# thu-ml/tianshou

Hardware: AMD Instinct MI355X
Metric: PPO learn() update-steps/sec (minibatch 65536, preprocessing incl.) + GAE transitions/sec; cpu_baseline / rocm_eager_baseline are PORTS of the reference path (oracle/), kind=port (higher is better)
Workload: dtype f32; 1 GPU; C2 PPO MuJoCo-shape rollout (BASELINE configs[1]): ONE rollout of 512 envs x 2048 steps = 2^20 transitions, minibatch 65536, obs 17, act 6, MLP[64,64] actor-critic, repeat 10, recompute_advantage off; parallelism=dp1, exchange=none

## Files before the change

### tianshou_amd/csrc/ts_ppo.hip

```cpp
#include <cstdlib>

#include "ts_common.h"

namespace {

using f32x16 = __attribute__((ext_vector_type(16))) float;
using f32x4 = __attribute__((ext_vector_type(4))) float;

constexpr int HID = 64;
constexpr int W2_PITCH = 68;
constexpr int W2_SIZE = HID * W2_PITCH;
constexpr int ACT_PAD = 8;
constexpr int TILE_PITCH = 36;
constexpr int TILE_SIZE = 32 * TILE_PITCH;
constexpr int STEP_THREADS = 256;
constexpr int STEP_WAVES = STEP_THREADS / 64;
constexpr int N_EXTRA = 2;

__device__ __forceinline__ int featF(int r, int h) { return (r & 3) + 8 * (r >> 2) + 4 * h; }

__device__ __forceinline__ f32x16 mfma32(float a, float b, f32x16 c) {
    return __builtin_amdgcn_mfma_f32_32x32x2f32(a, b, c, 0, 0, 0);
}

struct Dims {
    int obs, act;
    int a_w1, a_b1, a_w2, a_b2, a_wmu, a_bmu, a_sig, p_actor;
    int c_w1, c_b1, c_w2, c_b2, c_wv, c_bv, p_total;
};

__host__ __device__ inline Dims make_dims(int obs, int act) {
    Dims d;
    d.obs = obs; d.act = act;
    d.a_w1 = 0;
    d.a_b1 = d.a_w1 + HID * obs;
    d.a_w2 = d.a_b1 + HID;
    d.a_b2 = d.a_w2 + HID * HID;
    d.a_wmu = d.a_b2 + HID;
    d.a_bmu = d.a_wmu + act * HID;
    d.a_sig = d.a_bmu + act;
    d.p_actor = d.a_sig + act;
    d.c_w1 = d.p_actor;
    d.c_b1 = d.c_w1 + HID * obs;
    d.c_w2 = d.c_b1 + HID;
    d.c_b2 = d.c_w2 + HID * HID;
    d.c_wv = d.c_b2 + HID;
    d.c_bv = d.c_wv + HID;
    d.p_total = d.c_bv + 1;
    return d;
}

template <int KS1, int NN>
struct Lds {
    static constexpr int W2 = 0;
    static constexpr int W1 = W2 + NN * W2_SIZE;
    static constexpr int W1_NET = 2 * KS1 * HID;
    static constexpr int B2 = W1 + NN * W1_NET;
    static constexpr int WH = B2 + NN * HID;
    static constexpr int WH_NET = 2 * 2 * 16 * ACT_PAD;
    static constexpr int SMALL = WH + NN * WH_NET;
    static constexpr int END = SMALL + 32;
};

template <int NT, int COUNT, typename SrcFn, typename DstFn>
__device__ __forceinline__ void stage_batch(const float* __restrict__ params, float* lds, SrcFn src, DstFn dst) {
    constexpr int PER = (COUNT + NT - 1) / NT;
    float v[PER];
    int ok[PER];
#pragma unroll
    for (int k = 0; k < PER; ++k) {
        const int idx = threadIdx.x + NT * k;
        const int sidx = src(idx < COUNT ? idx : COUNT - 1);
        ok[k] = (idx < COUNT) & (sidx >= 0);
        v[k] = params[sidx >= 0 ? sidx : 0];
    }
#pragma unroll
    for (int k = 0; k < PER; ++k) v[k] = ok[k] ? v[k] : 0.f;
#pragma unroll
    for (int k = 0; k < PER; ++k) {
        const int idx = threadIdx.x + NT * k;
        if (idx < COUNT) lds[dst(idx)] = v[k];
    }
}

template <int KS1, int NN, int NT>
__device__ __forceinline__ void stage_weights(float* lds, const float* __restrict__ params,
                                              const Dims& d, int first_net) {
    using L = Lds<KS1, NN>;
    constexpr int N_W2 = HID * HID, N_W1 = 2 * KS1 * HID, N_B2 = HID, N_WH = L::WH_NET;
    constexpr int PER_NET = N_W2 + N_W1 + N_B2 + N_WH;
    constexpr int COUNT = NN * PER_NET + 32;
    const int obs = d.obs, act = d.act;
    auto src = [&](int idx) -> int {
        if (idx >= NN * PER_NET) {
            const int i = idx - NN * PER_NET;
            if (i < 8) return i < act ? d.a_bmu + i : -1;
            if (i < 24) return (i & 7) < act ? d.a_sig + (i & 7) : -1;
            return i == 24 ? d.c_bv : -1;
        }
        const int slot = idx / PER_NET;
        int i = idx - slot * PER_NET;
        const int net = first_net + slot;
        if (i < N_W2) return (net ? d.c_w2 : d.a_w2) + i;
        i -= N_W2;
        if (i < N_W1) {
            const int k = i >> 6, row = i & 63;
            const int w1 = net ? d.c_w1 : d.a_w1, b1 = net ? d.c_b1 : d.a_b1;
            return k < obs ? w1 + row * obs + k : (k == obs ? b1 + row : -1);
        }
        i -= N_W1;
        if (i < N_B2) return (net ? d.c_b2 : d.a_b2) + i;
        i -= N_B2;
        const int a = i & 7, r = (i >> 3) & 15, t = (i >> 7) & 1, h = (i >> 8) & 1;
        const int f = 32 * t + featF(r, h);
        if (net == 0) return a < act ? d.a_wmu + a * HID + f : -1;
        return a == 0 ? d.c_wv + f : -1;
    };
    auto dst = [&](int idx) -> int {
        if (idx >= NN * PER_NET) return L::SMALL + (idx - NN * PER_NET);
        const int slot = idx / PER_NET;
        int i = idx - slot * PER_NET;
        if (i < N_W2) return L::W2 + slot * W2_SIZE + (i >> 6) * W2_PITCH + (i & 63);
        i -= N_W2;
        if (i < N_W1) return L::W1 + slot * L::W1_NET + i;
        i -= N_W1;
        if (i < N_B2) return L::B2 + slot * HID + i;
        i -= N_B2;
        return L::WH + slot * L::WH_NET + i;
    };
    stage_batch<NT, COUNT>(params, lds, src, dst);
}

template <int KS1, int NN>
__device__ __forceinline__ void finish_small(float* lds) {
    using L = Lds<KS1, NN>;
    const int i = threadIdx.x;
    if (i >= 8 && i < 24) {
        const float sigma = expf(lds[L::SMALL + i]);
        lds[L::SMALL + i] = (i < 16) ? 1.f / (2.f * (sigma * sigma)) : logf(sigma);
    }
}

template <int KS1, int NT>
__device__ __forceinline__ void stage_image(float* lds, const float* __restrict__ img, int tid = threadIdx.x) {
    constexpr int N4 = Lds<KS1, 1>::END / 4, PER = (N4 + NT - 1) / NT;
    static_assert(Lds<KS1, 1>::END % 4 == 0, "image size");
    f32x4 v[PER];
#pragma unroll
    for (int k = 0; k < PER; ++k) {
        const int q = tid + NT * k;
        v[k] = reinterpret_cast<const f32x4*>(img)[q < N4 ? q : N4 - 1];
    }
#pragma unroll
    for (int k = 0; k < PER; ++k) {
        const int q = tid + NT * k;
        if (q < N4) reinterpret_cast<f32x4*>(lds)[q] = v[k];
    }
}

template <int KS1>
__global__ __launch_bounds__(256) void ppo_build_image_kernel(const float* __restrict__ params, Dims d,
                                                              float* __restrict__ image, int* __restrict__ inv) {
    using L = Lds<KS1, 1>;
    const int net = blockIdx.x;
    float* img = image + net * L::END;
    for (int i = threadIdx.x; i < L::END; i += 256) img[i] = 0.f;
    __syncthreads();
    stage_weights<KS1, 1, 256>(img, params, d, net);
    __syncthreads();
    finish_small<KS1, 1>(img);
    if (!inv) return;
    constexpr int N_W2 = HID * HID, N_W1 = 2 * KS1 * HID, N_B2 = HID, N_WH = L::WH_NET;
    constexpr int PER_NET = N_W2 + N_W1 + N_B2 + N_WH;
    for (int idx = threadIdx.x; idx < PER_NET + 32; idx += 256) {
        int src = -1, dst = -1;
        if (idx >= PER_NET) {
            const int i = idx - PER_NET;
            if (net == 0 && i < 8 && i < d.act) { src = d.a_bmu + i; dst = L::SMALL + i; }
            if (net == 1 && i == 24) { src = d.c_bv; dst = L::SMALL + 24; }
        } else {
            int i = idx;
            if (i < N_W2) { src = (net ? d.c_w2 : d.a_w2) + i; dst = L::W2 + (i >> 6) * W2_PITCH + (i & 63); }
            else if ((i -= N_W2) < N_W1) {
                const int k = i >> 6, row = i & 63;
                if (k < d.obs) src = (net ? d.c_w1 : d.a_w1) + row * d.obs + k;
                else if (k == d.obs) src = (net ? d.c_b1 : d.a_b1) + row;
                dst = L::W1 + i;
            } else if ((i -= N_W1) < N_B2) { src = (net ? d.c_b2 : d.a_b2) + i; dst = L::B2 + i; }
            else {
                i -= N_B2;
                const int a = i & 7, r = (i >> 3) & 15, t = (i >> 7) & 1, h = (i >> 8) & 1;
                const int f = 32 * t + featF(r, h);
                if (net == 0) { if (a < d.act) src = d.a_wmu + a * HID + f; }
                else if (a == 0) src = d.c_wv + f;
                dst = L::WH + i;
            }
        }
        if (src >= 0) inv[src] = net * L::END + dst;
    }
}

__device__ __forceinline__ float fast_tanh(float x) {
    const float e = __builtin_amdgcn_exp2f(x * 2.885390081777927f);
    return 1.f - 2.f * __builtin_amdgcn_rcpf(e + 1.f);
}

#ifndef TS_PK
#define TS_PK 2
#endif
using f32x2 = __attribute__((ext_vector_type(2))) float;
__device__ __forceinline__ void tanh16(f32x16& a) {
#if TS_PK < 1
#pragma unroll
    for (int r = 0; r < 16; ++r) a[r] = fast_tanh(a[r]);
    return;
#endif
#pragma unroll
    for (int r = 0; r < 16; r += 2) {
        const f32x2 x = {a[r], a[r + 1]};
        const f32x2 y = x * 2.885390081777927f;
        f32x2 e = {__builtin_amdgcn_exp2f(y[0]), __builtin_amdgcn_exp2f(y[1])};
        e = e + 1.f;
        const f32x2 q = {__builtin_amdgcn_rcpf(e[0]), __builtin_amdgcn_rcpf(e[1])};
        const f32x2 t = 1.f - 2.f * q;
        a[r] = t[0];
        a[r + 1] = t[1];
    }
}

__device__ __forceinline__ void dtanh16(f32x16& v, const f32x16& hh) {
#if TS_PK < 2
#pragma unroll
    for (int r = 0; r < 16; ++r) v[r] = v[r] * (1.f - hh[r] * hh[r]);
    return;
#endif
#pragma unroll
    for (int r = 0; r < 16; r += 2) {
        const f32x2 hv = {hh[r], hh[r + 1]};
        const f32x2 g = {v[r], v[r + 1]};
        const f32x2 o = g * (1.f - hv * hv);
        v[r] = o[0];
        v[r + 1] = o[1];
    }
}

template <int KS1, int NN>
__device__ __forceinline__ void trunk_forward(const float* lds, int net, const float (&x)[KS1],
                                              int i, int h, f32x16 (&h1)[2], f32x16 (&h2)[2]) {
    using L = Lds<KS1, NN>;
    const float* w1 = lds + L::W1 + net * L::W1_NET;
    const float* w2 = lds + L::W2 + net * W2_SIZE;
    const float* b2 = lds + L::B2 + net * HID;
#pragma unroll
    for (int t = 0; t < 2; ++t) {
        f32x16 acc = {0.f, 0.f, 0.f, 0.f, 0.f, 0.f, 0.f, 0.f, 0.f, 0.f, 0.f, 0.f, 0.f, 0.f, 0.f, 0.f};
#pragma unroll
        for (int s = 0; s < KS1; ++s) acc = mfma32(w1[(KS1 * h + s) * HID + 32 * t + i], x[s], acc);
        tanh16(acc);
        h1[t] = acc;
    }
#pragma unroll
    for (int t2 = 0; t2 < 2; ++t2) {
        f32x16 acc;
#pragma unroll
        for (int g = 0; g < 4; ++g) {
            const f32x4 b = *reinterpret_cast<const f32x4*>(b2 + 32 * t2 + 8 * g + 4 * h);
            acc[4 * g + 0] = b[0]; acc[4 * g + 1] = b[1]; acc[4 * g + 2] = b[2]; acc[4 * g + 3] = b[3];
        }
#pragma unroll
        for (int t = 0; t < 2; ++t) {
#pragma unroll
            for (int g = 0; g < 4; ++g) {
                const f32x4 a = *reinterpret_cast<const f32x4*>(w2 + (32 * t2 + i) * W2_PITCH + 32 * t + 8 * g + 4 * h);
#pragma unroll
                for (int q = 0; q < 4; ++q) acc = mfma32(a[q], h1[t][4 * g + q], acc);
            }
            __builtin_amdgcn_sched_barrier(0);
        }
        tanh16(acc);
        h2[t2] = acc;
    }
}

template <int KS1, int NN, int NA>
__device__ __forceinline__ void head_forward(const float* lds, int net, int h, const f32x16 (&h2)[2],
                                             float (&out)[NA]) {
    using L = Lds<KS1, NN>;
    const float* wh = lds + L::WH + net * L::WH_NET + h * (2 * 16 * ACT_PAD);
#pragma unroll
    for (int a = 0; a < NA; ++a) out[a] = 0.f;
#pragma unroll
    for (int t = 0; t < 2; ++t) {
#pragma unroll
        for (int r = 0; r < 16; ++r) {
            const float* p = wh + (t * 16 + r) * ACT_PAD;
            if constexpr (NA == 1) {
                out[0] += h2[t][r] * p[0];
            } else {
                const f32x4 w0 = *reinterpret_cast<const f32x4*>(p);
                const f32x4 w1 = *reinterpret_cast<const f32x4*>(p + 4);
#pragma unroll
                for (int a = 0; a < 4; ++a) {
                    out[a] += h2[t][r] * w0[a];
                    if (a + 4 < NA) out[a + 4] += h2[t][r] * w1[a];
                }
            }
            if (NA > 1 && (r & 7) == 7) __builtin_amdgcn_sched_barrier(0);
        }
    }
#pragma unroll
    for (int a = 0; a < NA; ++a) out[a] += __shfl_xor(out[a], 32, 64);
}

template <int KS1>
__device__ __forceinline__ void load_x(const float* __restrict__ obs, int64_t row, int obs_dim, int h,
                                       float (&x)[KS1]) {
#pragma unroll
    for (int s = 0; s < KS1; ++s) {
        const int k = KS1 * h + s;
        float v = 0.f;
        if (k < obs_dim) v = obs[row * obs_dim + k];
        else if (k == obs_dim) v = 1.f;
        x[s] = v;
    }
}

constexpr float LOG_SQRT_2PI = 0.91893853320467274178f;

__device__ __forceinline__ float gaussian_logp(const float (&mu)[ACT_PAD], const float (&act)[ACT_PAD],
                                               const float* sm, int act_dim) {
    float lp = 0.f;
#pragma unroll
    for (int a = 0; a < ACT_PAD; ++a) {
        if (a < act_dim) {
            const float dlt = act[a] - mu[a];
            lp += -(dlt * dlt) * sm[8 + a] - sm[16 + a] - LOG_SQRT_2PI;
        }
    }
    return lp;
}

template <int KS1>
__global__ __launch_bounds__(512) void ppo_infer_kernel(const float* __restrict__ params, Dims d,
                                                        const float* __restrict__ obs,
                                                        const float* __restrict__ act, int64_t n,
                                                        float* __restrict__ v_out,
                                                        float* __restrict__ logp_out,
                                                        float* __restrict__ mu_out, float mu_bound) {
    extern __shared__ __attribute__((aligned(16))) float lds[];
    using L = Lds<KS1, 2>;
    stage_weights<KS1, 2, 512>(lds, params, d, 0);
    __syncthreads();
    finish_small<KS1, 2>(lds);
    __syncthreads();
    const int lane = threadIdx.x & 63, i = lane & 31, h = lane >> 5;
    const int wave = threadIdx.x >> 6, waves = blockDim.x >> 6;
    const int64_t n_tiles = (n + 31) / 32;
    for (int64_t tile = (int64_t)blockIdx.x * waves + wave; tile < n_tiles; tile += (int64_t)gridDim.x * waves) {
        const int64_t srow = tile * 32 + i;
        const bool valid = srow < n;
        const int64_t row = valid ? srow : n - 1;
        float x[KS1];
        load_x<KS1>(obs, row, d.obs, h, x);
        f32x16 h1[2], h2[2];
        if (v_out) {
            trunk_forward<KS1, 2>(lds, 1, x, i, h, h1, h2);
            float v[1];
            head_forward<KS1, 2, 1>(lds, 1, h, h2, v);
            if (valid && h == 0) v_out[srow] = v[0] + lds[L::SMALL + 24];
        }
        if (logp_out || mu_out) {
            trunk_forward<KS1, 2>(lds, 0, x, i, h, h1, h2);
            float mu[ACT_PAD], a[ACT_PAD];
            head_forward<KS1, 2, ACT_PAD>(lds, 0, h, h2, mu);
#pragma unroll
            for (int k = 0; k < ACT_PAD; ++k) {
                mu[k] += lds[L::SMALL + k];
                if (mu_bound > 0.f) mu[k] = mu_bound * fast_tanh(mu[k]);
                a[k] = (logp_out && k < d.act) ? act[row * d.act + k] : 0.f;
            }
            if (mu_out && valid && h == 0) {
#pragma unroll
                for (int k = 0; k < ACT_PAD; ++k)
                    if (k < d.act) mu_out[srow * d.act + k] = mu[k];
            }
            if (logp_out) {
                const float lp = gaussian_logp(mu, a, lds + L::SMALL, d.act);
                if (valid && h == 0) logp_out[srow] = lp;
            }
        }
    }
}

struct StepArgs {
    const float* params;
    const float* rec;
    int rec_w;
    const int64_t* rows;
    int64_t n_rows;
    float inv_batch;
    const float* adv_stats;
    float eps_clip, dual_clip, vf_coef, ent_coef;
    int value_clip, adv_norm, a2c;
    int nets;
    float mu_bound;
    const float* image;
    float* slabs;
    int slab_w;
    long long* dbg;
};

#ifdef TS_PHASE_MARKS
#define TS_MARK(g, k)                                                                  \
    do {                                                                               \
        if ((g).dbg && blockIdx.x == 0 && threadIdx.x == 0) (g).dbg[(k)] = (long long)__builtin_readcyclecounter(); \
        if ((g).dbg && threadIdx.x == 0 && ((k) == 0 || (k) == 17))                    \
            (g).dbg[64 + 2 * blockIdx.x + ((k) == 17)] = (long long)__builtin_amdgcn_s_memrealtime();    \
        if ((g).dbg && threadIdx.x == 0 && (k) == 0)       \
            (g).dbg[64 + 1024 + blockIdx.x] = ((long long)__builtin_amdgcn_s_getreg((4 - 1) << 11 | 0 << 6 | 20) << 32) | \
                                              (unsigned)__builtin_amdgcn_s_getreg((32 - 1) << 11 | 0 << 6 | 4);          \
    } while (0)
#else
#define TS_MARK(g, k) do { } while (0)
#endif

__device__ __forceinline__ void tile_write(float* tile, const f32x16& v, int j, int h) {
#pragma unroll
    for (int r = 0; r < 16; ++r) tile[featF(r, h) * TILE_PITCH + j] = v[r];
}

__device__ __forceinline__ void wave_lds_sync() {
    __builtin_amdgcn_fence(__ATOMIC_ACQ_REL, "wavefront");
    __builtin_amdgcn_wave_barrier();
}

template <int KS1>
struct TileIn {
    float x[KS1];
    float act[ACT_PAD];
    float adv, logp_old, ret, v_old;
    float w;
};

template <int KS1>
struct RecFetch {
    static constexpr int N = (32 * ((2 * KS1 + 14) / 4) + 63) / 64;
    f32x4 v[N];
    float w;
};

struct RowId { int64_t id; float w; };

__device__ __forceinline__ RowId row_fetch(const StepArgs& g, int64_t tile, int lane) {
    const int i = lane & 31;
    const int64_t srow = tile * 32 + i;
    const bool valid = srow < g.n_rows;
    const int64_t pos = valid ? srow : g.n_rows - 1;
    RowId r;
    r.id = g.rows ? g.rows[pos] : pos;
    r.w = valid ? g.inv_batch : 0.f;
    return r;
}

template <int KS1>
__device__ __forceinline__ RecFetch<KS1> rec_fetch(const StepArgs& g, const RowId& row, int lane) {
    RecFetch<KS1> f;
    constexpr int REC_FETCH = RecFetch<KS1>::N;
    f.w = row.w;
    const int parts = g.rec_w >> 2;
    const int total = 32 * parts;
    const int lo = (int)(row.id & 0xffffffffLL), hi = (int)(row.id >> 32);
#pragma unroll
    for (int k = 0; k < REC_FETCH; ++k) {
        int q = lane + 64 * k;
        q = q < total ? q : total - 1;
        const int rec = q / parts, part = q - rec * parts;
        const int64_t rid = ((int64_t)__shfl(hi, rec, 64) << 32) | (uint32_t)__shfl(lo, rec, 64);
        f.v[k] = *reinterpret_cast<const f32x4*>(g.rec + rid * g.rec_w + part * 4);
    }
    return f;
}

template <int KS1>
__device__ __forceinline__ TileIn<KS1> rec_commit(const RecFetch<KS1>& f, const StepArgs& g, const Dims& d,
                                                   float* rb, int lane) {
    constexpr int REC_FETCH = RecFetch<KS1>::N;
    const int i = lane & 31, h = lane >> 5;
    const int parts = g.rec_w >> 2;
    const int total = 32 * parts;
#pragma unroll
    for (int k = 0; k < REC_FETCH; ++k) {
        const int q = lane + 64 * k;
        if (q < total) *reinterpret_cast<f32x4*>(rb + q * 4) = f.v[k];
    }
    wave_lds_sync();
    TileIn<KS1> t;
    const float* r = rb + i * g.rec_w;
#pragma unroll
    for (int s = 0; s < KS1; ++s) {
        const int k = KS1 * h + s;
        float v = 0.f;
        if (k < d.obs) v = r[k];
        else if (k == d.obs) v = 1.f;
        t.x[s] = v;
    }
#pragma unroll
    for (int k = 0; k < ACT_PAD; ++k) t.act[k] = (k < d.act) ? r[d.obs + k] : 0.f;
    const float* aux = r + d.obs + d.act;
    t.adv = aux[0];
    t.ret = aux[1];
    t.logp_old = aux[2];
    t.v_old = aux[3];
    t.w = f.w;
    wave_lds_sync();
    return t;
}

constexpr int P128 = 132;
constexpr int T2_FLOATS = 128 * P128;
constexpr int T2_XROW = 64;
constexpr int MISC_ROWS = 9;
constexpr int MISC_SLOT = MISC_ROWS * 64;
constexpr int T2_MISC = 96 * P128;
static_assert(T2_MISC + STEP_WAVES * MISC_SLOT <= T2_FLOATS, "misc slots must fit behind the phase-B tiles");

struct Slab2 {
    int w1[2], w2[2], b2[2], head[2], hb[2], sig, loss, width;
};

__host__ __device__ inline Slab2 slab2_layout(int act, int kp) {
    Slab2 L;
    int o = 0;
    for (int n = 0; n < 2; ++n) {
        const int n_head = n ? 1 : act;
        L.w1[n] = o; o += HID * kp;
        L.w2[n] = o; o += HID * HID;
        L.b2[n] = o; o += HID;
        L.head[n] = o; o += n_head * HID;
        L.hb[n] = o; o += n_head;
        if (n == 0) { L.sig = o; o += act; }
    }
    L.loss = o; o += N_EXTRA;
    L.width = (o + 3) & ~3;
    return L;
}

__device__ __forceinline__ int slab_col_to_param(int col, const Dims& d, int kp) {
    const Slab2 L = slab2_layout(d.act, kp);
    if (col >= L.loss) return col < L.loss + N_EXTRA ? d.p_total + (col - L.loss) : -1;
    const int n = col >= L.w1[1];
    const int c = col - L.w1[n];
    if (c < HID * kp) {
        const int f = c / kp, k = c - f * kp;
        const int w1 = n ? d.c_w1 : d.a_w1, b1 = n ? d.c_b1 : d.a_b1;
        return k < d.obs ? w1 + f * d.obs + k : (k == d.obs ? b1 + f : -1);
    }
    return (n ? d.c_w2 : d.a_w2) + (c - HID * kp);
}

__device__ __forceinline__ f32x4 ld4(const float* p) { return *reinterpret_cast<const f32x4*>(p); }

__device__ __forceinline__ void tile128_write(float* T, int row0, const f32x16& v, int col, int h) {
#pragma unroll
    for (int r = 0; r < 16; ++r) T[(row0 + featF(r, h)) * P128 + col] = v[r];
}

using gfloat_ptr = __attribute__((address_space(1))) float*;
#ifndef TS_SLAB_PLAIN_STORES
__device__ __forceinline__ void slab_st(float* p, float v) {
    __hip_atomic_store((gfloat_ptr)p, v, __ATOMIC_RELAXED, __HIP_MEMORY_SCOPE_AGENT);
}
#else
__device__ __forceinline__ void slab_st(float* p, float v) { *(gfloat_ptr)p = v; }
#endif

__device__ __forceinline__ void store_acc(float* p, float v, bool first) {
    if (!first) v += *(gfloat_ptr)p;
    slab_st(p, v);
}

template <bool WANT_RSUM>
__device__ __forceinline__ f32x16 tile128_mma(const float* T, int rowA, int rowB, int i, int h, float* rsum) {
    f32x16 c = {0.f, 0.f, 0.f, 0.f, 0.f, 0.f, 0.f, 0.f, 0.f, 0.f, 0.f, 0.f, 0.f, 0.f, 0.f, 0.f};
    const float* pa = T + (rowA + i) * P128 + 16 * h;
    const float* pb = T + (rowB + i) * P128 + 16 * h;
    float rs = 0.f;
    f32x4 a[4], b[4];
#pragma unroll
    for (int q = 0; q < 4; ++q) { a[q] = ld4(pa + 4 * q); b[q] = ld4(pb + 4 * q); }
#pragma unroll
    for (int ch = 0; ch < 4; ++ch) {
        f32x4 an[4], bn[4];
        if (ch < 3) {
#pragma unroll
            for (int q = 0; q < 4; ++q) { an[q] = ld4(pa + 32 * (ch + 1) + 4 * q); bn[q] = ld4(pb + 32 * (ch + 1) + 4 * q); }
        }
#pragma unroll
        for (int q = 0; q < 4; ++q) {
#pragma unroll
            for (int e = 0; e < 4; ++e) c = mfma32(a[q][e], b[q][e], c);
            if (WANT_RSUM) rs += (a[q][0] + a[q][1]) + (a[q][2] + a[q][3]);
        }
        if (ch < 3) {
#pragma unroll
            for (int q = 0; q < 4; ++q) { a[q] = an[q]; b[q] = bn[q]; }
        }
    }
    if (WANT_RSUM) *rsum = rs + __shfl_xor(rs, 32, 64);
    return c;
}

template <int KS1, bool ACTOR, bool BOUNDED = false>
__device__ __forceinline__ void net_fwd_bwd(float* lds, float* scratch, const StepArgs& g, const Dims& d,
                                            const TileIn<KS1>& in, int lane_in, f32x16 (&h1)[2], f32x16 (&h2)[2],
                                            f32x16 (&dz1)[2], float (&gw)[ACTOR ? ACT_PAD : 1], float& misc) {
    using L = Lds<KS1, 1>;
    int lane = lane_in;
    asm volatile("" : "+v"(lane));
    [[maybe_unused]] constexpr int MK = ACTOR ? 2 : 10;
    constexpr int NA = ACTOR ? ACT_PAD : 1;
    const int i = lane & 31, h = lane >> 5;
    trunk_forward<KS1, 1>(lds, 0, in.x, i, h, h1, h2);
    TS_MARK(g, MK + 0);

    float dout[NA];
    const float w = in.w;
    const float* sm = lds + L::SMALL;
    float* Qt = scratch;
    if constexpr (ACTOR) {
        float mu[ACT_PAD];
        head_forward<KS1, 1, ACT_PAD>(lds, 0, h, h2, mu);
        const f32x4 b0 = ld4(sm), b1 = ld4(sm + 4), v0 = ld4(sm + 8), v1 = ld4(sm + 12), s0 = ld4(sm + 16), s1 = ld4(sm + 20);
        float dlt[ACT_PAD], inv_var[ACT_PAD];
        [[maybe_unused]] float bgrad[ACT_PAD];
        constexpr bool bounded = BOUNDED;
        float logp = 0.f;
        int n_act = d.act;
        asm volatile("" : "+s"(n_act));
#pragma unroll
        for (int k = 0; k < ACT_PAD; ++k) {
            const float bm = k < 4 ? b0[k & 3] : b1[k & 3], iv = k < 4 ? v0[k & 3] : v1[k & 3], ls = k < 4 ? s0[k & 3] : s1[k & 3];
            float m = mu[k] + bm;
            if (bounded) {
                const float t = fast_tanh(m);
                m = g.mu_bound * t;
                bgrad[k] = 1.f - t * t;
            }
            dlt[k] = in.act[k] - m;
            inv_var[k] = 2.f * iv;
            logp += -(dlt[k] * dlt[k]) * iv - ls - (k < n_act ? LOG_SQRT_2PI : 0.f);
        }
        float mean = 0.f, den = 1.f;
        if (g.adv_norm) { mean = g.adv_stats[0]; den = g.adv_stats[1] + 1e-8f; }
        const float A = (in.adv - mean) / den;
        const bool a2c = g.a2c != 0;
        const float ratio = a2c ? 1.f : expf(logp - in.logp_old);
        const float surr1 = ratio * A;
        const float lo = 1.f - g.eps_clip, hi = 1.f + g.eps_clip;
        const float surr2 = fminf(fmaxf(ratio, lo), hi) * A;
        const float clip1 = fminf(surr1, surr2);
        float basek = (surr1 <= surr2) ? A : 0.f;
        const float dA = g.dual_clip * A;
        const bool dual = (g.dual_clip > 0.f) && (A < 0.f);
        float term = dual ? -fmaxf(clip1, dA) : -clip1;
        basek = (dual && !(clip1 >= dA)) ? 0.f : basek;
        term = a2c ? -logp * A : term;
        basek = a2c ? A : basek;
        const float dlogp = -basek * ratio * w;
        const float ent_w = g.ent_coef * w;
        float dsig[ACT_PAD];
#pragma unroll
        for (int k = 0; k < ACT_PAD; ++k) {
            dout[k] = dlogp * dlt[k] * inv_var[k];
            if (bounded) dout[k] = (dout[k] * g.mu_bound) * bgrad[k];
            const float ds = dlogp * (dlt[k] * dlt[k] * inv_var[k] - 1.f) - ent_w;
            dsig[k] = k < n_act ? ds : 0.f;
        }
#pragma unroll
        for (int k = 0; k < ACT_PAD; ++k) Qt[(8 * h + k) * TILE_PITCH + i] = h ? dsig[k] : dout[k];
        if (h == 0) Qt[16 * TILE_PITCH + i] = term * w;
    } else {
        float v[1];
        head_forward<KS1, 1, 1>(lds, 0, h, h2, v);
        const float value = v[0] + sm[24];
        const float ret = in.ret;
        const float vf1 = (ret - value) * (ret - value);
        const float vo = in.v_old;
        const float dvo = value - vo;
        const float vclip = vo + fminf(fmaxf(dvo, -g.eps_clip), g.eps_clip);
        const float vf2 = (ret - vclip) * (ret - vclip);
        const float g1 = -2.f * (ret - value);
        const float g2 = (dvo >= -g.eps_clip && dvo <= g.eps_clip) ? -2.f * (ret - vclip) : 0.f;
        const float dv_clip = (vf1 > vf2) ? g1 : ((vf2 > vf1) ? g2 : 0.5f * (g1 + g2));
        const bool vc = g.value_clip != 0;
        const float term = vc ? fmaxf(vf1, vf2) : vf1;
        const float dv = vc ? dv_clip : g1;
        dout[0] = dv * g.vf_coef * w;
        Qt[(16 * h) * TILE_PITCH + i] = h ? term * w : dout[0];
    }
    wave_lds_sync();
    {
        const int row = lane < 16 ? lane : 16;
        const float* rp = Qt + row * TILE_PITCH;
        f32x4 q[8];
#pragma unroll
        for (int k = 0; k < 8; ++k) q[k] = ld4(rp + 4 * k);
        float sacc = 0.f;
#pragma unroll
        for (int k = 0; k < 8; ++k) sacc += (q[k][0] + q[k][1]) + (q[k][2] + q[k][3]);
        const bool mine = ACTOR ? (lane <= 16) : (lane == 0 || lane == 16);
        misc = mine ? sacc : 0.f;
    }
    wave_lds_sync();
    __builtin_amdgcn_sched_barrier(0);
    TS_MARK(g, MK + 1);
    __builtin_amdgcn_s_setprio(ACTOR ? 2 : 0);

    float* SA = scratch;
    float* SB = scratch + TILE_SIZE;
    tile_write(SA, h2[0], i, h);
    tile_write(SB, h2[1], i, h);
    if (lane < 32) {
        if constexpr (ACTOR) {
            const f32x4 d0 = {dout[0], dout[1], dout[2], dout[3]};
            const f32x4 d1 = {dout[4], dout[5], dout[6], dout[7]};
            *reinterpret_cast<f32x4*>(SA + lane * TILE_PITCH + 32) = d0;
            *reinterpret_cast<f32x4*>(SB + lane * TILE_PITCH + 32) = d1;
        } else {
            SA[lane * TILE_PITCH + 32] = dout[0];
        }
    }
    wave_lds_sync();
    {
        const float* rowp = (lane < 32 ? SA : SB) + (lane & 31) * TILE_PITCH;
#pragma unroll
        for (int a = 0; a < NA; ++a) gw[a] = 0.f;
#pragma unroll 2
        for (int q = 0; q < 8; ++q) {
            const f32x4 hv = ld4(rowp + 4 * q);
#pragma unroll
            for (int e = 0; e < 4; ++e) {
                const int smp = 4 * q + e;
                if constexpr (ACTOR) {
                    const f32x4 d0 = ld4(SA + smp * TILE_PITCH + 32);
                    const f32x4 d1 = ld4(SB + smp * TILE_PITCH + 32);
#pragma unroll
                    for (int a = 0; a < 4; ++a) {
                        gw[a] += d0[a] * hv[e];
                        gw[a + 4] += d1[a] * hv[e];
                    }
                } else {
                    gw[0] += SA[smp * TILE_PITCH + 32] * hv[e];
                }
            }
        }
    }
    wave_lds_sync();
    __builtin_amdgcn_sched_barrier(0);
    TS_MARK(g, MK + 2);

    {
        const float* wh = lds + L::WH + h * (2 * 16 * ACT_PAD);
        [[maybe_unused]] f32x2 d01, d23, d45, d67;
        if constexpr (ACTOR) {
            d01 = f32x2{dout[0], dout[1]}; d23 = f32x2{dout[2], dout[3]};
            d45 = f32x2{dout[4], dout[5]}; d67 = f32x2{dout[6], dout[7]};
        }
#pragma unroll
        for (int t = 0; t < 2; ++t) {
            f32x16 dhv;
#pragma unroll
            for (int r = 0; r < 16; ++r) {
                const float* p = wh + (t * 16 + r) * ACT_PAD;
                if constexpr (ACTOR) {
                    const f32x4 w0 = ld4(p);
                    const f32x4 w1 = ld4(p + 4);
#if TS_PK < 3
                    dhv[r] = dout[0] * w0[0] + dout[1] * w0[1] + dout[2] * w0[2] + dout[3] * w0[3] +
                             dout[4] * w1[0] + dout[5] * w1[1] + dout[6] * w1[2] + dout[7] * w1[3];
                    continue;
#endif
                    f32x2 sacc = d01 * f32x2{w0[0], w0[1]};
                    sacc = d23 * f32x2{w0[2], w0[3]} + sacc;
                    sacc = d45 * f32x2{w1[0], w1[1]} + sacc;
                    sacc = d67 * f32x2{w1[2], w1[3]} + sacc;
                    dhv[r] = sacc[0] + sacc[1];
                } else {
                    dhv[r] = dout[0] * p[0];
                }
                if (ACTOR && (r & 7) == 7) __builtin_amdgcn_sched_barrier(0);
            }
            dtanh16(dhv, h2[t]);
            h2[t] = dhv;
        }
    }

    {
        const float* w2 = lds + L::W2;
#pragma unroll
        for (int t1 = 0; t1 < 2; ++t1) {
            f32x16 accd = {0.f, 0.f, 0.f, 0.f, 0.f, 0.f, 0.f, 0.f, 0.f, 0.f, 0.f, 0.f, 0.f, 0.f, 0.f, 0.f};
#pragma unroll
            for (int t = 0; t < 2; ++t) {
#pragma unroll
                for (int r = 0; r < 16; ++r)
                    accd = mfma32(w2[(32 * t + featF(r, h)) * W2_PITCH + 32 * t1 + i], h2[t][r], accd);
                __builtin_amdgcn_sched_barrier(0);
            }
            dtanh16(accd, h1[t1]);
            dz1[t1] = accd;
        }
    }
    __builtin_amdgcn_sched_barrier(0);
    TS_MARK(g, MK + 3);
}

template <int KS1, bool ACTOR>
__device__ __forceinline__ void net_wgrad(float* lds, const StepArgs& g, const Dims& d, const TileIn<KS1>& in,
                                          const f32x16 (&h1)[2], const f32x16 (&dz2)[2], const f32x16 (&dz1)[2],
                                          const float (&gw)[ACTOR ? ACT_PAD : 1], float misc, int wave, int lane_in,
                                          float* slab, const Slab2& SL, bool first) {
    [[maybe_unused]] constexpr int MK = ACTOR ? 2 : 10;
    constexpr int NA = ACTOR ? ACT_PAD : 1;
    constexpr int net = ACTOR ? 0 : 1;
    constexpr int KP = 2 * KS1;
    int lane = lane_in;
    asm volatile("" : "+v"(lane), "+v"(wave), "+s"(slab));
    const int i = lane & 31, h = lane >> 5;
    const int col = 32 * wave + i;
    float* T = lds;
    __syncthreads();
    tile128_write(T, 0, dz2[0], col, h);
    tile128_write(T, 32, dz2[1], col, h);
    tile128_write(T, 64, h1[0], col, h);
    tile128_write(T, 96, h1[1], col, h);
    __syncthreads();
    TS_MARK(g, MK + 4);
    {
        const int tM = wave >> 1, tN = wave & 1;
        float rs;
        const f32x16 c = tile128_mma<true>(T, 32 * tM, 64 + 32 * tN, i, h, &rs);
        float* p = slab + SL.w2[net] + (32 * tM + 4 * h) * HID + 32 * tN + i;
        if (first) {
#pragma unroll
            for (int r = 0; r < 16; ++r) slab_st(p + ((r & 3) + 8 * (r >> 2)) * HID, c[r]);
        } else {
#pragma unroll
            for (int r = 0; r < 16; ++r) slab_st(p + ((r & 3) + 8 * (r >> 2)) * HID, ((gfloat_ptr)p)[((r & 3) + 8 * (r >> 2)) * HID] + c[r]);
        }
        if (tN == 0 && h == 0) store_acc(slab + SL.b2[net] + 32 * tM + i, rs, first);
    }
    __syncthreads();
    TS_MARK(g, MK + 5);
    tile128_write(T, 0, dz1[0], col, h);
    tile128_write(T, 32, dz1[1], col, h);
#pragma unroll
    for (int s = 0; s < KS1; ++s) T[(T2_XROW + KS1 * h + s) * P128 + col] = in.x[s];
    {
        float* M = T + T2_MISC + wave * MISC_SLOT;
#pragma unroll
        for (int a = 0; a < NA; ++a) M[a * 64 + lane] = gw[a];
        M[8 * 64 + lane] = misc;
    }
    __syncthreads();
    const bool w1_wave = ACTOR ? (wave < 2) : (wave >= 2);
    if (w1_wave) {
        const int tM = wave & 1;
        const f32x16 c = tile128_mma<false>(T, 32 * tM, T2_XROW, i, h, nullptr);
        if (i < KP) {
            float* p = slab + SL.w1[net] + (32 * tM + 4 * h) * KP + i;
            if (first) {
#pragma unroll
                for (int r = 0; r < 16; ++r) slab_st(p + ((r & 3) + 8 * (r >> 2)) * KP, c[r]);
            } else {
#pragma unroll
                for (int r = 0; r < 16; ++r) slab_st(p + ((r & 3) + 8 * (r >> 2)) * KP, ((gfloat_ptr)p)[((r & 3) + 8 * (r >> 2)) * KP] + c[r]);
            }
        }
    } else {
        const int part = wave & 1;
        const float* M = T + T2_MISC;
        const int n_head = ACTOR ? d.act : 1;
        if (ACTOR) {
#pragma unroll
            for (int q = 0; q < 4; ++q) {
                const int row = 4 * part + q;
                float v = 0.f;
#pragma unroll
                for (int sl = 0; sl < STEP_WAVES; ++sl) v += M[sl * MISC_SLOT + row * 64 + lane];
                if (row < n_head) store_acc(slab + SL.head[net] + row * HID + lane, v, first);
            }
        } else if (part == 1) {
            float v = 0.f;
#pragma unroll
            for (int sl = 0; sl < STEP_WAVES; ++sl) v += M[sl * MISC_SLOT + lane];
            store_acc(slab + SL.head[net] + lane, v, first);
        }
        if (part == 0) {
            float v = 0.f;
#pragma unroll
            for (int sl = 0; sl < STEP_WAVES; ++sl) v += M[sl * MISC_SLOT + 8 * 64 + lane];
            if (lane < 8) { if (lane < n_head) store_acc(slab + SL.hb[net] + lane, v, first); }
            else if (lane < 16) { if (ACTOR && lane - 8 < d.act) store_acc(slab + SL.sig + lane - 8, v, first); }
            else if (lane == 16) store_acc(slab + SL.loss + net, v, first);
        }
    }
    TS_MARK(g, MK + 6);
}

template <int KS1, bool BOUNDED = false>
__global__ __launch_bounds__(STEP_THREADS, 2) void ppo_step2_kernel(StepArgs g, Dims d) {
    extern __shared__ __attribute__((aligned(16))) float lds[];
    using L = Lds<KS1, 1>;
    static_assert(L::END + STEP_WAVES * 2 * TILE_SIZE <= T2_FLOATS, "weight image + wave scratch must fit under the tiles");
    const int lane0 = threadIdx.x & 63, wave0 = threadIdx.x >> 6;
    const Slab2 SL = slab2_layout(d.act, 2 * KS1);

    const int64_t n_tiles = (g.n_rows + 31) / 32;
    const int64_t per_iter = (int64_t)gridDim.x * STEP_WAVES;
    const int64_t n_iter = (n_tiles + per_iter - 1) / per_iter;
    const int64_t tile0 = (int64_t)blockIdx.x * STEP_WAVES + wave0;
    float* slab = g.slabs + (int64_t)blockIdx.x * g.slab_w;

    TS_MARK(g, 0);
    for (int64_t it = 0; it < n_iter; ++it) {
        __builtin_amdgcn_s_setprio(3);
        int lane = lane0, wave = wave0;
        asm volatile("" : "+v"(lane), "+v"(wave));
        float* scratch = lds + L::END + wave * (2 * TILE_SIZE);
        const RowId row0 = row_fetch(g, it * per_iter + tile0, lane);
        const RecFetch<KS1> f = rec_fetch<KS1>(g, row0, lane);
        if (it > 0) __syncthreads();
        stage_image<KS1, STEP_THREADS>(lds, g.image, 64 * wave + lane);
        const TileIn<KS1> in = rec_commit<KS1>(f, g, d, scratch, lane);
        __syncthreads();
        TS_MARK(g, 1);
        const bool first = it == 0;
        f32x16 h1[2], h2[2], dz1[2];
        float misc;
        {
            float gw[ACT_PAD];
            net_fwd_bwd<KS1, true, BOUNDED>(lds, scratch, g, d, in, lane, h1, h2, dz1, gw, misc);
            net_wgrad<KS1, true>(lds, g, d, in, h1, h2, dz1, gw, misc, wave, lane, slab, SL, first);
        }
        __syncthreads();
        TS_MARK(g, 18);
        {
            int tid = 64 * wave + lane;
            asm volatile("" : "+v"(tid));
            stage_image<KS1, STEP_THREADS>(lds, g.image + L::END, tid);
        }
        __syncthreads();
        TS_MARK(g, 9);
        __builtin_amdgcn_s_setprio(1);
        {
            float gw[1];
            net_fwd_bwd<KS1, false>(lds, scratch, g, d, in, lane, h1, h2, dz1, gw, misc);
            net_wgrad<KS1, false>(lds, g, d, in, h1, h2, dz1, gw, misc, wave, lane, slab, SL, first);
        }
    }
    TS_MARK(g, 17);
}

template <int KS1, bool BOUNDED = false>
__global__ __launch_bounds__(STEP_THREADS, 2) void ppo_step1_kernel(StepArgs g, Dims d, int net) {
    extern __shared__ __attribute__((aligned(16))) float lds[];
    using L = Lds<KS1, 1>;
    const int lane0 = threadIdx.x & 63, wave0 = threadIdx.x >> 6;
    const Slab2 SL = slab2_layout(d.act, 2 * KS1);

    const int64_t n_tiles = (g.n_rows + 31) / 32;
    const int64_t per_iter = (int64_t)gridDim.x * STEP_WAVES;
    const int64_t n_iter = (n_tiles + per_iter - 1) / per_iter;
    const int64_t tile0 = (int64_t)blockIdx.x * STEP_WAVES + wave0;
    float* slab = g.slabs + (int64_t)blockIdx.x * g.slab_w;
    TS_MARK(g, 0);
    {
        const int z0 = net == 0 ? SL.w1[1] : 0, z1 = net == 0 ? SL.loss : SL.w1[1];
        for (int c = z0 + (int)threadIdx.x; c < z1; c += STEP_THREADS) slab_st(slab + c, 0.f);
        if (threadIdx.x == 0) slab_st(slab + SL.loss + (1 - net), 0.f);
    }
    for (int64_t it = 0; it < n_iter; ++it) {
        __builtin_amdgcn_s_setprio(3);
        int lane = lane0, wave = wave0;
        asm volatile("" : "+v"(lane), "+v"(wave));
        float* scratch = lds + L::END + wave * (2 * TILE_SIZE);
        const RowId row0 = row_fetch(g, it * per_iter + tile0, lane);
        const RecFetch<KS1> f = rec_fetch<KS1>(g, row0, lane);
        if (it > 0) __syncthreads();
        stage_image<KS1, STEP_THREADS>(lds, g.image + (net ? L::END : 0), 64 * wave + lane);
        const TileIn<KS1> in = rec_commit<KS1>(f, g, d, scratch, lane);
        __syncthreads();
        TS_MARK(g, 1);
        const bool first = it == 0;
        f32x16 h1[2], h2[2], dz1[2];
        float misc;
        if (net == 0) {
            float gw[ACT_PAD];
            net_fwd_bwd<KS1, true, BOUNDED>(lds, scratch, g, d, in, lane, h1, h2, dz1, gw, misc);
            net_wgrad<KS1, true>(lds, g, d, in, h1, h2, dz1, gw, misc, wave, lane, slab, SL, first);
        } else {
            float gw[1];
            net_fwd_bwd<KS1, false>(lds, scratch, g, d, in, lane, h1, h2, dz1, gw, misc);
            net_wgrad<KS1, false>(lds, g, d, in, h1, h2, dz1, gw, misc, wave, lane, slab, SL, first);
        }
    }
    TS_MARK(g, 17);
}

#include "ts_ppo_q.h"
#include "ts_npg_q.h"

constexpr int RED_THREADS = 1024;

__global__ __launch_bounds__(RED_THREADS) void ppo_reduce_slabs_kernel(const float* __restrict__ slabs,
                                                                       int n_slabs, int slab_w, Dims d, int kp, int k1q,
                                                                       float* __restrict__ grad,
                                                                       float* __restrict__ sumsq_part,
                                                                       const float* __restrict__ params,
                                                                       float* __restrict__ losses,
                                                                       float* __restrict__ parts) {
    __shared__ float red[RED_THREADS / 64][64];
    const int lane = threadIdx.x & 63, wave = threadIdx.x >> 6;
    const int col = blockIdx.x * 64 + lane;
    const int n_params = d.p_total;
    float s = 0.f;
    if (col < slab_w) {
#pragma unroll 16
        for (int k = wave; k < n_slabs; k += RED_THREADS / 64) s += slabs[(int64_t)k * slab_w + col];
    }
    red[wave][lane] = s;
    __syncthreads();
    if (wave == 0) {
        float t = 0.f;
#pragma unroll
        for (int k = 0; k < RED_THREADS / 64; ++k) t += red[k][lane];
        const int pidx = col < slab_w ? (k1q > 0 ? q4::slab3_col_to_param(col, d, k1q) : slab_col_to_param(col, d, kp)) : -1;
        if (pidx >= 0 && pidx < (parts ? n_params : n_params + N_EXTRA)) grad[pidx] = t;
        if (parts && pidx == n_params) parts[1] = t;
        if (parts && pidx == n_params + 1) parts[2] = t;
        float q = (pidx >= 0 && pidx < n_params) ? t * t : 0.f;
#pragma unroll
        for (int off = 32; off > 0; off >>= 1) q += __shfl_down(q, off, 64);
        if (lane == 0) sumsq_part[blockIdx.x] = q;
        if (parts && blockIdx.x == 0 && lane == 0) parts[0] = 0.f;
        if ((losses || parts) && blockIdx.x == 0 && lane == 0) {
            float ent = 0.f;
            for (int k = 0; k < d.act; ++k)
                ent += 0.5f + 0.5f * 1.8378770664093453f + logf(expf(params[d.a_sig + k]));
            if (losses) losses[3] = ent;
            if (parts) parts[3] = ent;
        }
    }
}

struct AdamArgs {
    float* params;
    float* m;
    float* v;
    const float* grad;
    const float* sumsq_part;
    int n_part, n_params;
    float max_grad_norm, lr_step, bc2_sqrt, beta1, beta2, eps;
    float omb1, omb2;
    float vf_coef, ent_coef;
    int opt_kind, centered;
    float wd, lr, alpha, oma, momentum;
    float* losses;
    int apply;
    float* image;
    const int* inv;
    int sig_off, act, small0;
};

constexpr int ADAM_THREADS = 256;

__global__ __launch_bounds__(ADAM_THREADS) void ppo_adam_kernel(AdamArgs a) {
    __shared__ float red[ADAM_THREADS / 64];
    const int tid = threadIdx.x, lane = tid & 63, wave = tid >> 6;
    const int p = blockIdx.x * ADAM_THREADS + tid;
    const bool mine = a.apply && p < a.n_params;
    const int pc = mine ? p : 0;
    float g_raw = a.grad[pc], m = a.m[pc], v = a.v[pc], par = a.params[pc];
    const int slot = (mine && a.image) ? a.inv[pc] : -1;
    float sq = 0.f;
    if (a.sumsq_part) {
        for (int k = tid; k < a.n_part; k += ADAM_THREADS) sq += a.sumsq_part[k];
    } else {
        for (int q = tid; q < a.n_params; q += ADAM_THREADS) { const float gq = a.grad[q]; sq += gq * gq; }
    }
#pragma unroll
    for (int off = 32; off > 0; off >>= 1) sq += __shfl_down(sq, off, 64);
    if (lane == 0) red[wave] = sq;
    __syncthreads();
    float total = 0.f;
#pragma unroll
    for (int k = 0; k < ADAM_THREADS / 64; ++k) total += red[k];
    const float norm = sqrtf(total);
    float scale = 1.f;
    if (a.max_grad_norm > 0.f) scale = fminf(a.max_grad_norm / (norm + 1e-6f), 1.f);

    if (a.losses && blockIdx.x == 0 && tid == 0) {
        const float clip = a.grad[a.n_params], vf = a.grad[a.n_params + 1];
        const float ent = a.losses[3];
        a.losses[0] = clip + a.vf_coef * vf - a.ent_coef * ent;
        a.losses[1] = clip;
        a.losses[2] = vf;
    }
    if (mine) {
        float gq = g_raw * scale;
        if (a.wd != 0.f) gq = gq + a.wd * par;
        float np_;
        if (a.opt_kind == TS_OPT_RMSPROP) {
            v = v * a.alpha + a.oma * gq * gq;
            float avg;
            if (a.centered) {
                m = m + (gq - m) * a.oma;
                avg = sqrtf(v + -1.f * m * m);
            } else {
                avg = sqrtf(v);
            }
            avg = avg + a.eps;
            if (a.momentum > 0.f) {
                m = m * a.momentum + gq / avg;
                np_ = par + -a.lr * m;
            } else {
                np_ = par + (-a.lr * gq) / avg;
            }
        } else {
            m = m + (gq - m) * a.omb1;
            v = v * a.beta2 + a.omb2 * gq * gq;
            const float denom = sqrtf(v) / a.bc2_sqrt + a.eps;
            np_ = par + (-a.lr_step * m) / denom;
        }
        a.params[p] = np_;
        a.m[p] = m;
        a.v[p] = v;
        if (a.image) {
            if (slot >= 0) a.image[slot] = np_;
            const int k = p - a.sig_off;
            if (k >= 0 && k < a.act) {
                const float sigma = expf(np_);
                a.image[a.small0 + 8 + k] = 1.f / (2.f * (sigma * sigma));
                a.image[a.small0 + 16 + k] = logf(sigma);
            }
        }
    }
}

__global__ __launch_bounds__(256) void ppo_pack_kernel(const float* __restrict__ obs,
                                                       const float* __restrict__ act,
                                                       const float* __restrict__ adv,
                                                       const float* __restrict__ ret,
                                                       const float* __restrict__ logp_old,
                                                       const float* __restrict__ v_old, int64_t n,
                                                       int obs_dim, int act_dim, int rec_w,
                                                       float* __restrict__ rec) {
    const int64_t total = n * rec_w;
    const int64_t stride = (int64_t)gridDim.x * blockDim.x;
    for (int64_t t = (int64_t)blockIdx.x * blockDim.x + threadIdx.x; t < total; t += stride) {
        const int64_t row = t / rec_w;
        const int c = (int)(t - row * rec_w);
        float v = 0.f;
        if (c < obs_dim) v = obs[row * obs_dim + c];
        else if (c < obs_dim + act_dim) v = act[row * act_dim + (c - obs_dim)];
        else if (c == obs_dim + act_dim) v = adv[row];
        else if (c == obs_dim + act_dim + 1) v = ret[row];
        else if (c == obs_dim + act_dim + 2) v = logp_old[row];
        else if (c == obs_dim + act_dim + 3) v = v_old[row];
        rec[t] = v;
    }
}

__global__ __launch_bounds__(1024) void ppo_adv_stats_kernel(const float* __restrict__ adv,
                                                             const int64_t* __restrict__ perm,
                                                             const int64_t* __restrict__ mb_offset,
                                                             float* __restrict__ out) {
    __shared__ double r1[16], r2[16];
    const int64_t lo = mb_offset[blockIdx.x], hi = mb_offset[blockIdx.x + 1];
    double s1 = 0.0, s2 = 0.0;
    for (int64_t k = lo + threadIdx.x; k < hi; k += 1024) {
        const double v = (double)adv[perm ? perm[k] : k];
        s1 += v;
        s2 += v * v;
    }
#pragma unroll
    for (int off = 32; off > 0; off >>= 1) {
        s1 += __shfl_down(s1, off, 64);
        s2 += __shfl_down(s2, off, 64);
    }
    if ((threadIdx.x & 63) == 0) { r1[threadIdx.x >> 6] = s1; r2[threadIdx.x >> 6] = s2; }
    __syncthreads();
    if (threadIdx.x == 0) {
        double t1 = 0.0, t2 = 0.0;
        for (int w = 0; w < 16; ++w) { t1 += r1[w]; t2 += r2[w]; }
        const double n = (double)(hi - lo);
        const double mean = t1 / n;
        const double var = (t2 - n * mean * mean) / (n - 1.0);
        out[2 * blockIdx.x] = (float)mean;
        out[2 * blockIdx.x + 1] = (float)sqrt(var > 0.0 ? var : 0.0);
    }
// ... 774 lines not shown
```

Measured before the change: 15580 update-steps/s.

## Split W1 gradient across all four waves using 16x16x4 MFMA tiles

The first-layer weight gradient used to be computed by two waves with 32x32x2 MFMA while the other two waves did the head and bias reductions. Now every wave computes a 16-row slice of dW1 with 16x16x4 MFMA, which only covers the padded K width instead of a full 32-wide tile. The head and bias reductions are redistributed by wave index. To match the new MFMA operand pattern, the LDS columns for dz1 and X are permuted. The aim is to balance work across waves and cut wasted MFMA lanes, at the cost of more complex LDS indexing and every wave doing both jobs.

```diff
diff --git a/tianshou_amd/csrc/ts_ppo.hip b/tianshou_amd/csrc/ts_ppo.hip
--- a/tianshou_amd/csrc/ts_ppo.hip
+++ b/tianshou_amd/csrc/ts_ppo.hip
@@ -21,6 +21,10 @@
 
 __device__ __forceinline__ f32x16 mfma32(float a, float b, f32x16 c) {
     return __builtin_amdgcn_mfma_f32_32x32x2f32(a, b, c, 0, 0, 0);
+}
+
+__device__ __forceinline__ f32x4 mfma16x4(float a, float b, f32x4 c) {
+    return __builtin_amdgcn_mfma_f32_16x16x4f32(a, b, c, 0, 0, 0);
 }
 
 struct Dims {
@@ -610,6 +614,43 @@
     return c;
 }
 
+__device__ __forceinline__ int dw1_col(int col) { return (col & ~15) | ((col & 1) << 3) | ((col & 15) >> 1); }
+
+template <int KS1>
+__device__ __forceinline__ void dw1_wave(const float* T, int wave, int lane, float* w1, bool first) {
+    constexpr int KP = 2 * KS1;
+    constexpr int NT = KP > 16 ? 2 : 1;
+    static_assert(KP <= 32 && T2_XROW + 16 * NT <= 96, "X^T rows stay below the misc slots");
+    const int m = lane & 15, kg = lane >> 4;
+    const int s0 = 16 * (kg & 1) + 8 * (kg >> 1);
+    const float* pa = T + (16 * wave + m) * P128 + s0;
+    const float* pb = T + (T2_XROW + m) * P128 + s0;
+    f32x4 acc[NT];
+#pragma unroll
+    for (int n = 0; n < NT; ++n) acc[n] = f32x4{0.f, 0.f, 0.f, 0.f};
+#pragma unroll
+    for (int t = 0; t < 8; ++t) {
+        const f32x4 a = ld4(pa + 32 * (t >> 1) + 4 * (t & 1));
+        f32x4 b[NT];
+#pragma unroll
+        for (int n = 0; n < NT; ++n) b[n] = ld4(pb + 16 * n * P128 + 32 * (t >> 1) + 4 * (t & 1));
+#pragma unroll
+        for (int e = 0; e < 4; ++e) {
+#pragma unroll
+            for (int n = 0; n < NT; ++n) acc[n] = mfma16x4(a[e], b[n][e], acc[n]);
+        }
+    }
+#pragma unroll
+    for (int n = 0; n < NT; ++n) {
+        const int k = 16 * n + m;
+        if (k < KP) {
+            float* p = w1 + (16 * wave + 4 * kg) * KP + k;
+#pragma unroll
+            for (int r = 0; r < 4; ++r) store_acc(p + r * KP, acc[n][r], first);
+        }
+    }
+}
+
 template <int KS1, bool ACTOR, bool BOUNDED = false>
 __device__ __forceinline__ void net_fwd_bwd(float* lds, float* scratch, const StepArgs& g, const Dims& d,
                                             const TileIn<KS1>& in, int lane_in, f32x16 (&h1)[2], f32x16 (&h2)[2],
@@ -823,7 +864,6 @@
     [[maybe_unused]] constexpr int MK = ACTOR ? 2 : 10;
     constexpr int NA = ACTOR ? ACT_PAD : 1;
     constexpr int net = ACTOR ? 0 : 1;
-    constexpr int KP = 2 * KS1;
     int lane = lane_in;
     asm volatile("" : "+v"(lane), "+v"(wave), "+s"(slab));
     const int i = lane & 31, h = lane >> 5;
@@ -852,10 +892,11 @@
     }
     __syncthreads();
     TS_MARK(g, MK + 5);
-    tile128_write(T, 0, dz1[0], col, h);
-    tile128_write(T, 32, dz1[1], col, h);
-#pragma unroll
-    for (int s = 0; s < KS1; ++s) T[(T2_XROW + KS1 * h + s) * P128 + col] = in.x[s];
+    const int colB = dw1_col(col);
+    tile128_write(T, 0, dz1[0], colB, h);
+    tile128_write(T, 32, dz1[1], colB, h);
+#pragma unroll
+    for (int s = 0; s < KS1; ++s) T[(T2_XROW + KS1 * h + s) * P128 + colB] = in.x[s];
     {
         float* M = T + T2_MISC + wave * MISC_SLOT;
 #pragma unroll
@@ -863,40 +904,26 @@
         M[8 * 64 + lane] = misc;
     }
     __syncthreads();
-    const bool w1_wave = ACTOR ? (wave < 2) : (wave >= 2);
-    if (w1_wave) {
-        const int tM = wave & 1;
-        const f32x16 c = tile128_mma<false>(T, 32 * tM, T2_XROW, i, h, nullptr);
-        if (i < KP) {
-            float* p = slab + SL.w1[net] + (32 * tM + 4 * h) * KP + i;
-            if (first) {
-#pragma unroll
-                for (int r = 0; r < 16; ++r) slab_st(p + ((r & 3) + 8 * (r >> 2)) * KP, c[r]);
-            } else {
-#pragma unroll
-                for (int r = 0; r < 16; ++r) slab_st(p + ((r & 3) + 8 * (r >> 2)) * KP, ((gfloat_ptr)p)[((r & 3) + 8 * (r >> 2)) * KP] + c[r]);
-            }
-        }
-    } else {
-        const int part = wave & 1;
+    dw1_wave<KS1>(T, wave, lane, slab + SL.w1[net], first);
+    {
         const float* M = T + T2_MISC;
         const int n_head = ACTOR ? d.act : 1;
         if (ACTOR) {
 #pragma unroll
-            for (int q = 0; q < 4; ++q) {
-                const int row = 4 * part + q;
+            for (int q = 0; q < 2; ++q) {
+                const int row = 2 * wave + q;
                 float v = 0.f;
 #pragma unroll
                 for (int sl = 0; sl < STEP_WAVES; ++sl) v += M[sl * MISC_SLOT + row * 64 + lane];
                 if (row < n_head) store_acc(slab + SL.head[net] + row * HID + lane, v, first);
             }
-        } else if (part == 1) {
+        } else if (wave == 1) {
             float v = 0.f;
 #pragma unroll
             for (int sl = 0; sl < STEP_WAVES; ++sl) v += M[sl * MISC_SLOT + lane];
             store_acc(slab + SL.head[net] + lane, v, first);
         }
-        if (part == 0) {
+        if (wave == 0) {
             float v = 0.f;
 #pragma unroll
             for (int sl = 0; sl < STEP_WAVES; ++sl) v += M[sl * MISC_SLOT + 8 * 64 + lane];
```

New measurement: 16230 update-steps/s (median of 6 runs). 1.04x the previous value.
